# ka9q/ka9q-radio

Hardware: NVIDIA H100
Metric: input Msamples/s through forward+filter+inverse at N channels (higher is better)
Workload: dtype f32

## Files before the change

include/ka9q_gpu.h:

```cpp
#ifndef KA9Q_GPU_H
#define KA9Q_GPU_H 1
#include <stddef.h>
#include <stdint.h>

#ifdef __cplusplus
extern "C" {
#endif

enum kgpu_type { KGPU_COMPLEX = 1, KGPU_REAL = 2 };
enum kgpu_format {
  KGPU_FMT_F32 = 0,
  KGPU_FMT_I16 = 1
};
enum kgpu_chan_flags {
  KGPU_CHAN_ISB = 1,
  KGPU_CHAN_BEAM = 4
};

typedef struct kgpu_master kgpu_master;
typedef struct kgpu_bank kgpu_bank;

struct kgpu_ingest_stats {
  unsigned long long energy;
  unsigned int clips;
// ... 136 lines not shown
int kgpu_bank_run_one_ex(kgpu_bank *b, int idx, const void *d_spec, void *d_out, float *d_power , void *stream);
int kgpu_bank_noise(kgpu_bank *b, const void *d_spec, int nblocks, double samprate, double *d_n0, void *stream);

int kgpu_bank_fm_front(kgpu_bank *b, const void *d_out, long out_pitch, int nblocks, float *d_baseband, double *d_stats, void *stream);

int kgpu_bank_commit(kgpu_bank *b, void *stream);
int kgpu_use_static_kernels(int on);
int kgpu_use_cols_tma(int on);
int kgpu_cols_tma_fits(int L, int M, int in_type, int fmt, const void *d_in);
int kgpu_use_fused_forward(int on);
int kgpu_fused_forward_fits(int L, int M, int in_type, int fmt, const void *d_in);
int kgpu_fused_forward_options(int lead, int discard);
int kgpu_fused_shape(int *out);
int kgpu_fused_schedule(int nblocks, int lead, int ticket, int *out);
long kgpu_fused_discards(int blk, int idx, long *lines, long max);

int kgpu_plan_radices(int len, int *radices, int max);
int kgpu_plan_split(long n, int *n1, int *n2);
int kgpu_plan_radices_ex(int len, int *radices, int max);
int kgpu_plan_split_ex(long n, int *n1, int *n2);

int kgpu_multicast_copy(const void *d_src, void *mc_dst, unsigned long long bytes, int nctas, void *stream);

typedef struct kgpu_spectrum kgpu_spectrum;
kgpu_spectrum *kgpu_spectrum_create(int fft_n, int in_type, int bin_count);
int kgpu_spectrum_set_window(kgpu_spectrum *s, float const *window);
int kgpu_spectrum_run(kgpu_spectrum *s, const void *d_ring, long ring_samples, long end, int fmt, float scale,
                      const struct kgpu_scale_change *d_chg, int nchg, long long end_index, int derandomize, int shift, int fft_avg, double overlap, float *d_bins, void *stream);
int kgpu_spectrum_run_narrow(kgpu_spectrum *s, const void *d_ring, long ring_size, long ring_idx, int fft_avg,
                             double overlap, float *d_bins, int *fft_avg_used, void *stream);
// ... 12 lines not shown
```

ka9q_radio_b200/capi.py:

```python
from __future__ import annotations

import ctypes as C
import os
import subprocess
from pathlib import Path

PKG = Path(__file__).resolve().parent
LIB_PATH = PKG / "libka9qgpu.so"

KGPU_COMPLEX, KGPU_REAL = 1, 2
KGPU_FMT_F32, KGPU_FMT_I16 = 0, 1
KGPU_RAW_U8, KGPU_RAW_S8 = 1, 2
KGPU_RAW_S16, KGPU_RAW_U16, KGPU_RAW_SC16Q11 = 3, 4, 5
KGPU_RAW_F32, KGPU_RAW_CF32, KGPU_RAW_CF32_CNRMF, KGPU_RAW_CF32_FSCALE = 6, 7, 8, 9
KGPU_CHAN_ISB = 1
KGPU_CHAN_BEAM = 4

_lib = None


class KgpuError(RuntimeError):
    pass


# ... 81 lines not shown
    L.kgpu_bank_block_counter.restype = l
    L.kgpu_bank_run_ex.argtypes = [vp, vp, i, vp, l, vp, vp]
    L.kgpu_bank_run_one_ex.argtypes = [vp, i, vp, vp, vp, vp]
    L.kgpu_bank_noise.argtypes = [vp, vp, i, d, vp, vp]
    L.kgpu_bank_fm_front.argtypes = [vp, vp, l, i, vp, vp, vp]
    L.kgpu_use_static_kernels.argtypes = [i]
    L.kgpu_use_cols_tma.argtypes = [i]
    L.kgpu_cols_tma_fits.argtypes = [i, i, i, i, vp]
    L.kgpu_use_fused_forward.argtypes = [i]
    L.kgpu_fused_forward_fits.argtypes = [i, i, i, i, vp]
    L.kgpu_fused_forward_options.argtypes = [i, i]
    L.kgpu_fused_shape.argtypes = [vp]
    L.kgpu_fused_schedule.argtypes = [i, i, i, vp]
    L.kgpu_fused_discards.argtypes = [i, i, vp, l]
    L.kgpu_fused_discards.restype = l
    L.kgpu_profile_enable.argtypes = [i]
    L.kgpu_profile_name.argtypes = [i]
    L.kgpu_profile_name.restype = C.c_char_p
    L.kgpu_profile_get.argtypes = [i, vp, vp]
    L.kgpu_plan_radices.argtypes = [i, vp, i]
    L.kgpu_plan_split.argtypes = [l, vp, vp]
    L.kgpu_plan_radices_ex.argtypes = [i, vp, i]
    L.kgpu_plan_split_ex.argtypes = [l, vp, vp]
    L.kgpu_multicast_copy.argtypes = [vp, vp, C.c_ulonglong, i, vp]
    L.kgpu_algorithmic_bytes.argtypes = [vp, vp, i]
    L.kgpu_algorithmic_bytes.restype = d
    L.kgpu_spectrum_create.restype = vp
    L.kgpu_spectrum_create.argtypes = [i, i, i]
    L.kgpu_spectrum_set_window.argtypes = [vp, vp]
    L.kgpu_spectrum_run.argtypes = [vp, vp, l, l, i, f, vp, i, C.c_longlong, i, i, i, d, vp, vp]
# ... 369 lines not shown
```

ka9q_radio_b200/csrc/fft_static.cuh:

```cuda
#pragma once
#include "fft_radix.cuh"

namespace kfft {

template <int LEN, int... RS> struct SPlan {
  static constexpr int len = LEN;
  static constexpr int nst = sizeof...(RS);
  static constexpr int rad_arr[sizeof...(RS) > 0 ? sizeof...(RS) : 1] = {RS...};
  static constexpr int rad(int i) { return rad_arr[i]; }
  static constexpr int nsub(int i) {
    int n = LEN;
    for (int k = 0; k < i; k++) n /= rad_arr[k];
    return n;
  }
  static constexpr int stride(int i) { return nsub(i) / rad_arr[i]; }
  static constexpr int tw_off(int i) {
    int o = 0;
    for (int k = 0; k < i; k++)
      if (stride(k) > 1) o += (rad_arr[k] - 1) * stride(k);
    return o;
  }
  static constexpr bool valid() {
    int p = 1;
    for (int k = 0; k < nst; k++) p *= rad_arr[k];
// ... 104 lines not shown
}
__device__ __forceinline__ void mbar_fence_init() { asm volatile("fence.mbarrier_init.release.cluster;" ::: "memory"); }
__device__ __forceinline__ void mbar_expect_tx(uint64_t *bar, uint32_t bytes) {
  asm volatile("mbarrier.arrive.expect_tx.shared::cta.b64 _, [%0], %1;" ::"r"(smem_u32(bar)), "r"(bytes) : "memory");
}
__device__ __forceinline__ void bulk_g2s(void *dst, void const *src, uint32_t bytes, uint64_t *bar) {
  asm volatile("cp.async.bulk.shared::cluster.global.mbarrier::complete_tx::bytes [%0], [%1], %2, [%3];" ::"r"(smem_u32(dst)),
               "l"(src), "r"(bytes), "r"(smem_u32(bar))
               : "memory");
}
__device__ __forceinline__ void tensor_g2s_3d(void *dst, void const *map, int x, int y, int z, uint64_t *bar) {
  asm volatile("cp.async.bulk.tensor.3d.shared::cluster.global.tile.mbarrier::complete_tx::bytes [%0], [%1, {%2, %3, %4}], [%5];"
               ::"r"(smem_u32(dst)), "l"(map), "r"(x), "r"(y), "r"(z), "r"(smem_u32(bar))
               : "memory");
}
__device__ __forceinline__ void fence_proxy_async_global() { asm volatile("fence.proxy.async.global;" ::: "memory"); }
__device__ __forceinline__ void discard_l2_line(void *p) { asm volatile("discard.global.L2 [%0], 128;" ::"l"(p) : "memory"); }
__device__ __forceinline__ void mbar_wait(uint64_t *bar, uint32_t parity) {
  asm volatile(
      "{\n\t.reg .pred p;\n\t"
      "WAIT_%=:\n\t"
      "mbarrier.try_wait.parity.shared::cta.b64 p, [%0], %1;\n\t"
      "@p bra DONE_%=;\n\t"
      "bra WAIT_%=;\n\t"
      "DONE_%=:\n\t}" ::"r"(smem_u32(bar)),
      "r"(parity)
      : "memory");
}

}
// ... 1 lines not shown
```

ka9q_radio_b200/csrc/fwd_fused.cuh:

```cuda
#pragma once
#include "fwd_cols_r36.cuh"
#include "static_kernels_v2.cuh"

namespace kfft {

struct FusedShape {
  static constexpr int N1 = 1296, N2 = 1250;
  static constexpr int TILES = (N2 + 7) / 8;
  static constexpr int NC = (TILES + 1) / 2;
  static constexpr int NR = (N1 / 2 + 1 + RowsV2Shape<true>::IPC - 1) / RowsV2Shape<true>::IPC;
  static constexpr int T = 2 * ColsR36Shape::T;
  static constexpr int RT = RowsV2Shape<true>::T;
  static constexpr size_t smem = 2 * ColsR36Shape::smem > RowsV2Shape<true>::smem ? 2 * ColsR36Shape::smem : RowsV2Shape<true>::smem;
  static constexpr int DEFAULT_LEAD = 40;
  static_assert(ColsR36Shape::smem % 16 == 0, "the second tile's memory 16-byte aligned");
  static_assert(T % 32 == 0 && ColsR36Shape::T % 32 == 0 && RT % 32 == 0, "whole warps per tile and per R item");
};

enum FusedKind : int { kFusedCol = 0, kFusedRow = 1 };
struct FusedItem {
  int kind, blk, idx;
};

__host__ __device__ __forceinline__ FusedItem fused_item(int t, int nblocks, int lead) {
  using F = FusedShape;
  if (t < F::NC) return {kFusedCol, 0, t};
  t -= F::NC;
  int const b = t / (F::NR + F::NC), p = t - b * (F::NR + F::NC);
// ... 10 lines not shown
  int discard;
};

__device__ __forceinline__ void red_release_gpu_add(unsigned *p, unsigned v) {
  asm volatile("red.release.gpu.global.add.u32 [%0], %1;" ::"l"(p), "r"(v) : "memory");
}
__device__ __forceinline__ unsigned ld_acquire_gpu(unsigned const *p) {
  unsigned v;
  asm volatile("ld.acquire.gpu.global.u32 %0, [%1];" : "=r"(v) : "l"(p) : "memory");
  return v;
}

template <int FMT>
__global__ void __launch_bounds__(FusedShape::T, 1)
    fwd_fused_r36_v2(Pass1Args const a1, ColsR36Tables const t1, Pass2Args const a2, FwdTables const t2, FusedArgs const f,
                     const __grid_constant__ CUtensorMap tmap) {
  using F = FusedShape;
  extern __shared__ __align__(16) unsigned char smem_raw[];
  __shared__ __align__(8) uint64_t bars[RowsV2Shape<true>::COLS];
  __shared__ __align__(8) uint64_t tbar[2];
  __shared__ int s_ticket;
  int const tid = threadIdx.x;
  if (tid == 0) s_ticket = (int)atomicAdd(f.ctr, 1u);
  __syncthreads();
  FusedItem const it = fused_item(s_ticket, f.nblocks, f.lead);
  if (it.kind == kFusedCol) {
    int const h = tid >= ColsR36Shape::T, tile = 2 * it.idx + h;
    if (tile < F::TILES)
      fwd_cols_r36_body<FMT, F::N2, true>(a1, t1, &tmap, smem_raw + h * ColsR36Shape::smem, tbar[h], tid - h * ColsR36Shape::T,
                                           tile * 8, it.blk, [h] {
                                             asm volatile("bar.sync %0, %1;" ::"r"(1 + h), "n"(ColsR36Shape::T) : "memory");
// ... 6 lines not shown
    return;
  }
  if (tid >= F::RT) return;
  auto sync = [] { asm volatile("bar.sync 3, %0;" ::"n"(F::RT) : "memory"); };
  auto sync_or = [](int p) {
    int r;
    asm volatile("{\n\t.reg .pred q, o;\n\tsetp.ne.s32 q, %1, 0;\n\tbar.red.or.pred o, 3, %2, q;\n\tselp.s32 %0, 1, 0, o;\n\t}"
                 : "=r"(r)
                 : "r"(p), "n"(F::RT)
                 : "memory");
    return r;
  };
  if (tid == 0)
    while (ld_acquire_gpu(f.ctr + 1 + it.blk) < (unsigned)F::NC) __nanosleep(64);
  sync();
  fwd_rows_v2_body<true, F::N1, true, true>(a2, t2, smem_raw, bars, tbar[0], tid, it.blk, it.idx * RowsV2Shape<true>::IPC,
                                            sync, sync_or, f.discard);
}

}
```

ka9q_radio_b200/csrc/fwd_kernels.cuh:

```cuda
#pragma once
#include "fft_tile.cuh"

namespace kfft {

constexpr int kTile = 8;
constexpr int kFwdThreads = kTile * 32;

struct IngestStats {
  unsigned long long energy;
  unsigned int clips;
  unsigned int pad;
};

struct Pass1Args {
  void const *in;
  long hop;
  int n1, n2;
  long nc;
  int plan;
  int pitch;
  float scale;
  int derandomize;
  long first_new;
  float2 *mid;
// ... 146 lines not shown
  else it.kind = kRowEmpty, it.row_a = it.row_b = 0;
  return it;
}

struct Pass2Args {
  float2 const *mid;
  int n1, n2;
  long nc;
  int plan;
  int pitch;
  int real_split;
  float2 const *rootD;
  float2 *spec;
  long spec_stride;
  int mid_ld;
};

__global__ void __launch_bounds__(kFwdThreads, 2) fwd_rows_kernel(Pass2Args const a) {
  TilePlan const &pl = c_plans[a.plan];
#define KFFT_ROWS_EXT false
#include "fwd_rows_body.cuh"
#undef KFFT_ROWS_EXT
}
__global__ void __launch_bounds__(kFwdThreads, 2) fwd_rows_ext(Pass2Args const a, __grid_constant__ TilePlan const pl) {
#define KFFT_ROWS_EXT true
#include "fwd_rows_body.cuh"
#undef KFFT_ROWS_EXT
}

struct NotchDev {
// ... 34 lines not shown
```

ka9q_radio_b200/csrc/kgpu.cu:

```cuda
#include <cuda_runtime.h>
#include <cudaTypedefs.h>
#include <math.h>
#include <stdarg.h>
#include <stdio.h>
#include <stdlib.h>
#include <string.h>
#include <algorithm>
#include <complex>
#include <atomic>
#include <map>
#include <mutex>
#include <string>
#include <vector>

#include "../../include/ka9q_gpu.h"
#include "chan_kernels.cuh"
#include "chan_huge.cuh"
#include "chan_wide.cuh"
#include "fwd_kernels.cuh"
#include "noise_kernel.cuh"
#include "plan.cuh"
#include "static_kernels.cuh"
#include "static_kernels_v2.cuh"
#include "fwd_cols_r36.cuh"
// ... 30 lines not shown
  }
  return v != 0;
}
static std::atomic<int> g_fused{-1};
static std::atomic<int> g_fused_lead{FusedShape::DEFAULT_LEAD}, g_fused_discard{0};
extern "C" int kgpu_use_fused_forward(int on) {
  g_fused.store(on != 0);
  return 0;
}
static bool fused_on() {
  int v = g_fused.load();
  if (v < 0) {
    char const *e = getenv("KA9Q_FUSED_FWD");
    g_fused.compare_exchange_strong(v, (e && *e) ? (atoi(e) != 0) : 1);
    v = g_fused.load();
  }
  return v != 0;
}

static int fail(char const *fmt, ...) {
  char buf[512];
  va_list ap;
  va_start(ap, fmt);
  vsnprintf(buf, sizeof buf, fmt, ap);
  va_end(ap);
  g_err = buf;
  return -1;
}
#define CUDA_OK(expr)                                                                    \
  do {                                                                                   \
// ... 893 lines not shown
  size_t smem1 = 0, smem2 = 0;
  bool ext = false;
  TilePlan xplan1{}, xplan2{};
  kgpu_master *bs = nullptr;
  Bluestein blue;
  StreamBuf b_in, b_out;
  int b_chunk = 0;
  NotchDev *d_notch = nullptr;
  int n_notch = 0;
  int notch_sequential = 0;
};

using ColsR36Fn = void (*)(Pass1Args, ColsR36Tables);
using ColsR36TmaFn = void (*)(Pass1Args, ColsR36Tables, CUtensorMap);
using Cols2sFn = void (*)(Pass1Args, Cols2sTables);
using RowsV2Fn = void (*)(Pass2Args, FwdTables);
using Cols2s = Cols2sShape<25, 32>;
using Rows2s = Rows2sShape<25, 25>;
static ColsR36Fn cols_r36_kernel(kgpu_master const *m, int f) {
  static ColsR36Fn const k[2][3] = {{fwd_cols_r36<0, 0>, fwd_cols_r36<1, 0>, fwd_cols_r36<2, 0>},
                                    {fwd_cols_r36<0, 1250>, fwd_cols_r36<1, 1250>, fwd_cols_r36<2, 1250>}};
  return k[m->n2c == 1250][f];
}
static ColsR36TmaFn cols_r36_tma_kernel(kgpu_master const *m, int f) {
  static ColsR36TmaFn const k[2][3] = {{fwd_cols_r36_tma<0, 0>, fwd_cols_r36_tma<1, 0>, fwd_cols_r36_tma<2, 0>},
                                       {fwd_cols_r36_tma<0, 1250>, fwd_cols_r36_tma<1, 1250>, fwd_cols_r36_tma<2, 1250>}};
  return k[m->n2c == 1250][f];
}
static Cols2sFn cols_2s_kernel(int f) {
  static Cols2sFn const k[3] = {fwd_cols_2s<0, 25, 32>, fwd_cols_2s<1, 25, 32>, fwd_cols_2s<2, 25, 32>};
  return k[f];
}
static RowsV2Fn rows_v2_kernel(kgpu_master const *m) {
  if (m->in_type == KGPU_REAL) return m->halved ? fwd_rows_v2<true, 1296, true> : fwd_rows_v2<true, 0, false>;
  return m->n1c ? fwd_rows_v2<false, 1296, false> : fwd_rows_v2<false, 0, false>;
}
static bool fused_pair(kgpu_master const *m) {
  return m->in_type == KGPU_REAL && m->cols == COLS_R36 && m->rows == ROWS_V2 && m->halved && m->n2c == FusedShape::N2 &&
         m->n1c == FusedShape::N1 && m->mid_ld % 16 == 0;
}
using FusedFn = void (*)(Pass1Args, ColsR36Tables, Pass2Args, FwdTables, FusedArgs, CUtensorMap);
static FusedFn fused_kernel(int f) {
  static FusedFn const k[3] = {fwd_fused_r36_v2<0>, fwd_fused_r36_v2<1>, fwd_fused_r36_v2<2>};
  return k[f];
}
static int rows_v2_threads(kgpu_master const *m) { return m->in_type == KGPU_REAL ? RowsV2Shape<true>::T : RowsV2Shape<false>::T; }
static size_t rows_v2_smem(kgpu_master const *m) {
  return m->in_type == KGPU_REAL ? RowsV2Shape<true>::smem : RowsV2Shape<false>::smem;
}

static int upload(float2 **d, std::vector<float2> const &v) {
  CUDA_OK(cudaMalloc(d, sizeof(float2) * v.size()));
  CUDA_OK(cudaMemcpy(*d, v.data(), sizeof(float2) * v.size(), cudaMemcpyHostToDevice));
  return 0;
}

static int bluestein_upload(Bluestein *b) {
  if (upload(&b->d_b, bluestein_bspec(b->n, b->P)) == 0) return 0;
  cudaFree(b->d_b);
  b->d_b = nullptr;
  return -1;
}

// ... 78 lines not shown
    std::vector<float2> t0((size_t)Cols2s::TW0, make_float2(0.f, 0.f)), tA((size_t)n2 * RA),
        tB((size_t)(n2 + 8) * Cols2s::NP1, make_float2(0.f, 0.f)), r0((size_t)Rows2s::TW0, make_float2(0.f, 0.f));
    for (int e = 0; e < Cols2s::NP0; e++)
      for (int j = 0; j < RB; j++) t0[(size_t)e * RB + j] = root((long)j * Pow<RA>::exponent(e), n1);
    for (long c = 0; c < n2; c++) {
      for (int t = 0; t < RA; t++) tA[(size_t)c * RA + t] = root(c * t, m->nc);
      for (int e = 0; e < Cols2s::NP1; e++) tB[(size_t)c * Cols2s::NP1 + e] = root(c * RA * Pow<RB>::exponent(e), m->nc);
    }
    for (int e = 0; e < Rows2s::NP0; e++)
      for (int j = 0; j < RD; j++) r0[(size_t)e * RD + j] = root((long)j * Pow<RC>::exponent(e), n2);
    if (upload(&m->d_tw0, t0) || upload(&m->d_twA, tA) || upload(&m->d_twB, tB) || upload(&m->d_rtw0, r0)) return -1;
    for (int f = 0; f < 3; f++)
      if (allow_smem((const void *)cols_2s_kernel(f), Cols2s::smem)) return -1;
    if (allow_smem((const void *)fwd_rows_2s<25, 25>, Rows2s::smem)) return -1;
  }
  if (m->rows == ROWS_V2 && allow_smem((const void *)rows_v2_kernel(m), rows_v2_smem(m))) return -1;
  if (fused_pair(m))
    for (int f = 0; f < 3; f++)
      if (allow_smem((const void *)fused_kernel(f), FusedShape::smem)) return -1;
  if (m->ext) {
    if (allow_smem((const void *)fwd_cols_ext<0>, m->smem1) || allow_smem((const void *)fwd_cols_ext<1>, m->smem1) ||
        allow_smem((const void *)fwd_rows_ext, m->smem2))
      return -1;
  } else if (allow_smem((const void *)fwd_cols_kernel<0>, m->smem1) || allow_smem((const void *)fwd_cols_kernel<1>, m->smem1) ||
             allow_smem((const void *)fwd_rows_kernel, m->smem2)) {
    return -1;
  }
  return 0;
}

extern "C" void kgpu_master_destroy(kgpu_master *m) {
  if (!m) return;
  if (m->ext) {
    free_tile_plan(m->xplan1);
// ... 231 lines not shown
extern "C" long kgpu_fused_discards(int blk, int idx, long *lines, long max) {
  using S = RowsV2Shape<true>;
  if (blk < 0 || idx < 0 || idx >= FusedShape::NR || max < 0) return fail("kgpu_fused_discards: bad arguments");
  int const ld = (FusedShape::N2 + 15) / 16 * 16;
  long n = 0;
  for (int col = 0; col < S::COLS; col++) {
    RowItem const it = row_item(idx * S::IPC + (col >> 1), FusedShape::N1, true);
    int const row = (col & 1) == 0 ? (it.kind != kRowEmpty ? it.row_a : -1) : (it.kind == kRowPair ? it.row_b : -1);
    if (row < 0) continue;
    for (int l = 0; l < mid_row_lines(ld); l++, n++)
      if (lines && n < max) lines[n] = mid_line(blk, FusedShape::N1, row, ld, l);
  }
  return n;
}

static int cols_tma_map(kgpu_master const *m, void const *d_in, int fmt, int nblocks, CUtensorMap *map) {
  static PFN_cuTensorMapEncodeTiled const encode = [] {
    void *fn = nullptr;
    cudaDriverEntryPointQueryResult q;
    if (cudaGetDriverEntryPoint("cuTensorMapEncodeTiled", &fn, cudaEnableDefault, &q) != cudaSuccess ||
        q != cudaDriverEntryPointSuccess)
      fn = nullptr;
    return (PFN_cuTensorMapEncodeTiled)fn;
  }();
  if (!encode) return fail("kgpu_forward: the driver has no cuTensorMapEncodeTiled");
  bool const i16 = fmt == KGPU_FMT_I16;
  cuuint64_t const n1 = (cuuint64_t)m->sp.n1, n2 = (cuuint64_t)m->sp.n2;
  cuuint64_t const hop = (cuuint64_t)(m->in_type == KGPU_REAL ? m->L / 2 : m->L);
  cuuint64_t const dim[3] = {2 * n2, i16 ? n1 / 2 : n1, (cuuint64_t)nblocks};
  cuuint64_t const stride[2] = {8 * n2, hop * (i16 ? 4 : 8)};
  cuuint32_t const box[3] = {(cuuint32_t)(i16 ? ColsR36Tma::I16_BOX_WORDS : 16), ColsR36Tma::BOX_ROWS, 1};
  cuuint32_t const unit[3] = {1, 1, 1};
  CUresult const r = encode(map, i16 ? CU_TENSOR_MAP_DATA_TYPE_UINT32 : CU_TENSOR_MAP_DATA_TYPE_FLOAT32, 3, const_cast<void *>(d_in),
                            dim, stride, box, unit, CU_TENSOR_MAP_INTERLEAVE_NONE, CU_TENSOR_MAP_SWIZZLE_NONE,
                            CU_TENSOR_MAP_L2_PROMOTION_L2_128B, CU_TENSOR_MAP_FLOAT_OOB_FILL_NONE);
  if (r != CUDA_SUCCESS) return fail("kgpu_forward: cuTensorMapEncodeTiled failed (%d)", (int)r);
  return 0;
}

static Pass2Args rows_args(kgpu_master const *m, Pass1Args const &a1, void *d_spec) {
  Pass2Args a2;
  a2.mid = a1.mid;
  a2.n1 = m->sp.n1;
  a2.n2 = m->sp.n2;
  a2.nc = m->nc;
  a2.plan = m->plan2;
  a2.pitch = m->pitch2;
  a2.real_split = (m->in_type == KGPU_REAL);
  a2.rootD = m->d_rootD;
  a2.spec = (float2 *)d_spec;
  a2.spec_stride = m->spec_stride;
  a2.mid_ld = a1.mid_ld;
  return a2;
}

static int fused_span(kgpu_master *m, const void *d_in, int fmt, int f, int nblocks, void *d_spec, cudaStream_t st,
                      Pass1Args const &a1) {
  using F = FusedShape;
  size_t const ctr_bytes = sizeof(unsigned) * (size_t)(1 + nblocks);
  if (grow(m->fused_ctr, ctr_bytes, st, "kgpu_forward")) return -1;
  CUtensorMap map;
  if (cols_tma_map(m, d_in, fmt, nblocks, &map)) return -1;
  FusedArgs fa;
  fa.ctr = (unsigned *)m->fused_ctr.p;
  fa.nblocks = nblocks;
  fa.lead = g_fused_lead.load();
  fa.discard = g_fused_discard.load();
  CUDA_OK(cudaMemsetAsync(fa.ctr, 0, ctr_bytes, st));
  {
    ProfScope ps(K_FWD_FUSED, st);
    fused_kernel(f)<<<(unsigned)(nblocks * (F::NC + F::NR)), F::T, F::smem, st>>>(a1, ColsR36Tables{m->d_tw0, m->d_twA, m->d_twB},
                                                                       rows_args(m, a1, d_spec), FwdTables{m->d_rootC}, fa, map);
  }
  g_launches++;
  CUDA_OK(cudaGetLastError());
  return 0;
}

static int forward_span(kgpu_master *m, const void *d_in, int fmt, float scale, int derandomize, int nblocks, void *d_spec,
                        void *d_stats, cudaStream_t st, float2 *mid) {
  bool const use_static = g_static_on.load() != 0;
  ColsKernel const cols = use_static ? m->cols : COLS_GENERIC;
  RowsKernel const rows = use_static ? m->rows : ROWS_GENERIC;
  Pass1Args a1;
  a1.in = d_in;
  a1.hop = (m->in_type == KGPU_REAL) ? m->L / 2 : m->L;
  a1.n1 = m->sp.n1;
// ... 23 lines not shown
          if (cols_tma_map(m, d_in, fmt, nblocks, &map)) return -1;
          cols_r36_tma_kernel(m, f)<<<g1, ColsR36Shape::T, ColsR36Shape::smem, st>>>(a1, ColsR36Tables{m->d_tw0, m->d_twA, m->d_twB}, map);
        } else {
          cols_r36_kernel(m, f)<<<g1, ColsR36Shape::T, ColsR36Shape::smem, st>>>(a1, ColsR36Tables{m->d_tw0, m->d_twA, m->d_twB});
        }
        break;
      case COLS_GENERIC:
        if (m->ext && f) fwd_cols_ext<1><<<g1, kFwdThreads, m->smem1, st>>>(a1, m->xplan1);
        else if (m->ext) fwd_cols_ext<0><<<g1, kFwdThreads, m->smem1, st>>>(a1, m->xplan1);
        else if (f) fwd_cols_kernel<1><<<g1, kFwdThreads, m->smem1, st>>>(a1);
        else fwd_cols_kernel<0><<<g1, kFwdThreads, m->smem1, st>>>(a1);
        break;
    }
  }
  g_launches++;
  Pass2Args const a2 = rows_args(m, a1, d_spec);
  dim3 const g2((unsigned)(rows == ROWS_GENERIC ? m->n_item_ctas : m->n_rows_ctas), (unsigned)nblocks);
  {
    ProfScope ps(K_FWD_ROWS, st);
    switch (rows) {
      case ROWS_2S:
        fwd_rows_2s<25, 25><<<g2, Rows2s::T, Rows2s::smem, st>>>(a2, m->d_rtw0);
        break;
      case ROWS_V2:
        rows_v2_kernel(m)<<<g2, rows_v2_threads(m), rows_v2_smem(m), st>>>(a2, FwdTables{m->d_rootC});
        break;
      case ROWS_GENERIC:
        if (m->ext) fwd_rows_ext<<<g2, kFwdThreads, m->smem2, st>>>(a2, m->xplan2);
        else fwd_rows_kernel<<<g2, kFwdThreads, m->smem2, st>>>(a2);
        break;
    }
  }
  g_launches++;
  CUDA_OK(cudaGetLastError());
  return 0;
}

static int bluestein_conv(kgpu_master *im, Bluestein const &b, float2 *a, int rows, float2 *y, cudaStream_t st) {
  if (kgpu_forward(im, a, KGPU_FMT_F32, 1.0f, 0, rows, y, nullptr, st) != 0) return -1;
  {
// ... 1336 lines not shown
```

ka9q_radio_b200/csrc/static_kernels_v2.cuh:

```cuda
#pragma once
#include "static_kernels.cuh"

namespace kfft {

__device__ __forceinline__ void unpack_i16(int raw, int &lo, int &hi) {
  asm("prmt.b32 %0, %1, 0, 0x9910;" : "=r"(lo) : "r"(raw));
  hi = raw >> 16;
}
__device__ __forceinline__ float i32_to_f32(int v) {
  float f;
  asm("cvt.rn.f32.s32 %0, %1;" : "=f"(f) : "r"(v));
  return f;
}

template <bool REAL_SPLIT>
struct RowsV2Shape {
  using P = SPlan<1250, 10, 25, 5>;
  static constexpr int N2 = 1250, PITCH = 1250, GT = 256, SKEW = 2;
  static constexpr int NG = REAL_SPLIT ? 2 : 1, T = GT * NG, COLS = 8 * NG;
  static constexpr int IPC = REAL_SPLIT ? COLS / 2 : COLS;
  static constexpr int TW = (static_tw_count<P>() + 1) & ~1;
  static constexpr int TILE = COLS * PITCH + (NG - 1) * SKEW;
  static constexpr size_t smem = sizeof(float2) * (size_t)(TILE + TW);
  static __host__ __device__ constexpr int col_off(int c) { return c * PITCH + (c >> 3) * SKEW; }
};

__device__ constexpr float kRowsTw0[3][4][2] = {
    {{9.870916009e-01f, -1.601568460e-01f}, {9.486995935e-01f, -3.161789477e-01f}, {8.000617623e-01f, -5.999176502e-01f}, {2.801976204e-01f, -9.599423409e-01f}},
    {{9.486995935e-01f, -3.161789477e-01f}, {8.000617623e-01f, -5.999176502e-01f}, {2.801976204e-01f, -9.599423409e-01f}, {-8.429785967e-01f, -5.379471183e-01f}},
    {{8.858151436e-01f, -4.640382826e-01f}, {5.693368912e-01f, -8.221042752e-01f}, {-3.517109454e-01f, -9.361086488e-01f}, {-7.525988221e-01f, 6.584793329e-01f}},
};

__host__ __device__ constexpr int mid_row_lines(int mid_ld) { return mid_ld * 8 / 128; }
__host__ __device__ constexpr long mid_line(int blk, int n1, int row, int mid_ld, int l) {
  return ((long)blk * n1 + row) * mid_row_lines(mid_ld) + l;
}

template <bool REAL_SPLIT, int N1C, bool HALVED, bool FUSED, class Sync, class SyncOr>
__device__ __forceinline__ void fwd_rows_v2_body(Pass2Args const &a, FwdTables const &tb, unsigned char *smem_raw,
                                                 uint64_t *bars, uint64_t &tbar, int tid, int blk, int item0,
                                                 Sync const &sync, SyncOr const &sync_or, bool discard = false) {
  using S = RowsV2Shape<REAL_SPLIT>;
  using P = typename S::P;
  constexpr int N2 = S::N2, T = S::T, GT = S::GT, COLS = S::COLS, IPC = S::IPC;
  constexpr int R0 = 10, S0 = 125, R1 = 25, NSUB1 = 125, S1 = 5, R2 = 5;
  float2 *tile = reinterpret_cast<float2 *>(smem_raw);
  float2 *s_tw = tile + S::TILE;
  TilePlan const &pl = c_plans[a.plan];
  int const lane = tid & 31, warp = tid >> 5;
  int const n1 = N1C ? N1C : a.n1;
  auto row_of = [&](int col) -> int {
    RowItem const it = row_item(item0 + (REAL_SPLIT ? col >> 1 : col), n1, REAL_SPLIT);
    if (REAL_SPLIT) {
      if ((col & 1) == 0) return it.kind != kRowEmpty ? it.row_a : -1;
      return it.kind == kRowPair ? it.row_b : -1;
    }
// ... 63 lines not shown
    float2 const *tw1 = s_tw + P::tw_off(1);
#pragma unroll 1
    for (int u = ul; u < N2 / R1; u += GT / 8) {
      int const b = u / S1, j = u - b * S1;
      float2 *p = mycol + b * NSUB1 + j;
      float2 x[R1];
#pragma unroll
      for (int m = 0; m < R1; m++) x[m] = p[m * S1];
      Dft<R1, false>::run(x);
#pragma unroll
      for (int t = 1; t < R1; t++) x[t] = cmul(x[t], tw1[(t - 1) * S1 + j]);
#pragma unroll
      for (int t = 0; t < R1; t++) p[t * S1] = x[t];
    }
  }
  constexpr int UQ = T / IPC;
  int const i = tid % IPC, uq = tid / IPC;
  RowItem const it = row_item(item0 + i, n1, REAL_SPLIT);
  float2 rootC = make_float2(1.f, 0.f), rd[4];
  bool self_item = false;
  if (REAL_SPLIT) {
    self_item = it.kind == kRowSelf0 || it.kind == kRowSelfMid;
    if (it.kind == kRowPair) rootC = __ldg(tb.rootC + it.row_a);
#pragma unroll
    for (int q = 0; q < 4; q++) {
      int const u = uq + UQ * q;
      int const t0 = u / 25, t1 = u - t0 * 25;
      rd[q] = (it.kind == kRowPair && u < N2 / R2) ? __ldg(a.rootD + t0 + 10 * t1) : make_float2(1.f, 0.f);
    }
  }
  int const has_self = sync_or(self_item);

  float2 *spec = a.spec + (long)blk * a.spec_stride;
  float const hf = HALVED ? 1.0f : 0.5f;
  if (!REAL_SPLIT) {
    if (col_ok) {
      float2 *dst = spec + row_of(c);
#pragma unroll 1
      for (int u = ul; u < N2 / R2; u += GT / 8) {
        int const t0 = u / 25, t1 = u - t0 * 25;
        int const kb = t0 + 10 * t1;
        float2 const *p = mycol + u * R2;
        float2 x[R2];
#pragma unroll
        for (int m = 0; m < R2; m++) x[m] = p[m];
        Dft<R2, false>::run(x);
        float2 *d = dst + (long)n1 * kb;
#pragma unroll
        for (int t = 0; t < R2; t++) d[(long)n1 * 250 * t] = x[t];
      }
    }
    return;
  }
  int const nc = N1C ? N1C * N2 : (int)a.nc;
  if (it.kind == kRowPair) {
    float2 const *ca = tile + S::col_off(2 * i), *cb = tile + S::col_off(2 * i + 1);
#pragma unroll
    for (int q = 0; q < 4; q++) {
      int const u = uq + UQ * q;
      if (u >= N2 / R2) break;
      int const t0 = u / 25, t1 = u - t0 * 25;
      int const kb = t0 + 10 * t1;
      float2 const wkb = cmul(rootC, rd[q]);
      float2 za[R2], zb[R2];
      float2 const *pa = ca + u * R2, *pb = cb + (N2 / R2 - 1 - u) * R2;
      float2 *pk = spec + (it.row_a + n1 * kb), *pm = spec + (nc - it.row_a - n1 * kb);
#pragma unroll
      for (int m = 0; m < R2; m++) {
        za[m] = pa[m];
        zb[m] = pb[m];
      }
      Dft<R2, false>::run(za);
      Dft<R2, false>::run(zb);
#pragma unroll
      for (int t = 0; t < R2; t++) {
        float2 const A = za[t], B = zb[R2 - 1 - t];
        float2 const w = (t == 0) ? wkb : cmul(wkb, wroot<10>(t));
        float2 const E = HALVED ? make_float2(A.x + B.x, A.y - B.y) : make_float2(0.5f * (A.x + B.x), 0.5f * (A.y - B.y));
        float2 const O = HALVED ? make_float2(A.x - B.x, A.y + B.y) : make_float2(0.5f * (A.x - B.x), 0.5f * (A.y + B.y));
        float2 const Pp = cmul(w, O);
        pk[(long)n1 * 250 * t] = make_float2(E.x + Pp.y, E.y - Pp.x);
        pm[-(long)n1 * 250 * t] = make_float2(E.x - Pp.y, -(E.y + Pp.x));
      }
    }
  }
  if (!has_self) return;
  for (int s = 0; s < IPC; s++) {
    RowItem const its = row_item(item0 + s, n1, true);
    if (its.kind != kRowSelf0 && its.kind != kRowSelfMid) continue;
    float2 *col = tile + S::col_off(2 * s);
    for (int u = tid; u < N2 / R2; u += T) {
      float2 x[R2];
#pragma unroll
      for (int m = 0; m < R2; m++) x[m] = col[u * R2 + m];
      Dft<R2, false>::run(x);
#pragma unroll
      for (int m = 0; m < R2; m++) col[u * R2 + m] = x[m];
// ... 10 lines not shown
    for (int k2 = tid; k2 < kend; k2 += T) {
      int const k2m = self0 ? (k2 == 0 ? 0 : N2 - k2) : N2 - 1 - k2;
      float2 const A = col[static_slot<P>(k2)], B = col[static_slot<P>(k2m)];
      float2 const w = cmul(rC, __ldg(a.rootD + k2));
      float2 const E = make_float2(hf * (A.x + B.x), hf * (A.y - B.y));
      float2 const O = make_float2(hf * (A.x - B.x), hf * (A.y + B.y));
      float2 const Pp = cmul(w, O);
      int const k = its.row_a + n1 * k2;
      spec[k] = make_float2(E.x + Pp.y, E.y - Pp.x);
      if (nc - k != k) spec[nc - k] = make_float2(E.x - Pp.y, -(E.y + Pp.x));
    }
  }
}

template <bool REAL_SPLIT, int N1C = 0, bool HALVED = false>
__global__ void __launch_bounds__(RowsV2Shape<REAL_SPLIT>::T, REAL_SPLIT ? 1 : 2) fwd_rows_v2(Pass2Args const a, FwdTables const tb) {
  extern __shared__ __align__(16) unsigned char smem_raw[];
  __shared__ __align__(8) uint64_t bars[RowsV2Shape<REAL_SPLIT>::COLS];
  __shared__ __align__(8) uint64_t tbar;
  fwd_rows_v2_body<REAL_SPLIT, N1C, HALVED, false>(a, tb, smem_raw, bars, tbar, threadIdx.x, gridDim.y - 1 - blockIdx.y,
                                                   blockIdx.x * RowsV2Shape<REAL_SPLIT>::IPC, [] { __syncthreads(); },
                                                   [](int p) { return __syncthreads_or(p); });
}

template <class P, bool OSC = false>
__global__ void __launch_bounds__(kChanWarps * 32) chan_v2(ChanArgs const a) {
  static_assert(P::nst == 2, "two-stage plans only");
  __shared__ __align__(8) uint64_t bars[kChanWarps];
  __shared__ __align__(8) uint64_t tbar;
  using S = StaticChan<P>;
  constexpr int NS = S::NS, R0 = P::rad(0), R1 = P::rad(1), S0 = NS / R0;
  static_assert(S0 == R1, "plan shape");
  S s;
  if (!static_prologue<P>(a, bars, tbar, s)) return;
  ChanDesc const &d = s.d;
// ... 52 lines not shown
```

Baseline: 104,100.

## Store forward rows-pass low-half spectrum via TMA bulk tensor stores

```diff
diff --git a/include/ka9q_gpu.h b/include/ka9q_gpu.h
--- a/include/ka9q_gpu.h
+++ b/include/ka9q_gpu.h
@@ -174,6 +174,8 @@
 int kgpu_fused_shape(int *out);
 int kgpu_fused_schedule(int nblocks, int lead, int ticket, int *out);
 long kgpu_fused_discards(int blk, int idx, long *lines, long max);
+int kgpu_use_rows_tma_store(int on);
+int kgpu_rows_store_box(int item, int round, int *out);
 
 int kgpu_plan_radices(int len, int *radices, int max);
 int kgpu_plan_split(long n, int *n1, int *n2);
diff --git a/ka9q_radio_b200/capi.py b/ka9q_radio_b200/capi.py
--- a/ka9q_radio_b200/capi.py
+++ b/ka9q_radio_b200/capi.py
@@ -119,6 +119,8 @@
     L.kgpu_fused_schedule.argtypes = [i, i, i, vp]
     L.kgpu_fused_discards.argtypes = [i, i, vp, l]
     L.kgpu_fused_discards.restype = l
+    L.kgpu_use_rows_tma_store.argtypes = [i]
+    L.kgpu_rows_store_box.argtypes = [i, i, vp]
     L.kgpu_profile_enable.argtypes = [i]
     L.kgpu_profile_name.argtypes = [i]
     L.kgpu_profile_name.restype = C.c_char_p
diff --git a/ka9q_radio_b200/csrc/fft_static.cuh b/ka9q_radio_b200/csrc/fft_static.cuh
--- a/ka9q_radio_b200/csrc/fft_static.cuh
+++ b/ka9q_radio_b200/csrc/fft_static.cuh
@@ -142,6 +142,15 @@
                ::"r"(smem_u32(dst)), "l"(map), "r"(x), "r"(y), "r"(z), "r"(smem_u32(bar))
                : "memory");
 }
+__device__ __forceinline__ void tensor_s2g_4d(void const *map, void const *src, int x, int y, int z, int w) {
+  asm volatile("cp.async.bulk.tensor.4d.global.shared::cta.bulk_group [%0, {%1, %2, %3, %4}], [%5];" ::"l"(map), "r"(x), "r"(y),
+               "r"(z), "r"(w), "r"(smem_u32(src))
+               : "memory");
+}
+__device__ __forceinline__ void bulk_commit() { asm volatile("cp.async.bulk.commit_group;" ::: "memory"); }
+__device__ __forceinline__ void bulk_wait_read_all() { asm volatile("cp.async.bulk.wait_group.read 0;" ::: "memory"); }
+__device__ __forceinline__ void bulk_wait_all() { asm volatile("cp.async.bulk.wait_group 0;" ::: "memory"); }
+__device__ __forceinline__ void fence_proxy_async_shared() { asm volatile("fence.proxy.async.shared::cta;" ::: "memory"); }
 __device__ __forceinline__ void fence_proxy_async_global() { asm volatile("fence.proxy.async.global;" ::: "memory"); }
 __device__ __forceinline__ void discard_l2_line(void *p) { asm volatile("discard.global.L2 [%0], 128;" ::"l"(p) : "memory"); }
 __device__ __forceinline__ void mbar_wait(uint64_t *bar, uint32_t parity) {
diff --git a/ka9q_radio_b200/csrc/fwd_fused.cuh b/ka9q_radio_b200/csrc/fwd_fused.cuh
--- a/ka9q_radio_b200/csrc/fwd_fused.cuh
+++ b/ka9q_radio_b200/csrc/fwd_fused.cuh
@@ -12,6 +12,7 @@
   static constexpr int T = 2 * ColsR36Shape::T;
   static constexpr int RT = RowsV2Shape<true>::T;
   static constexpr size_t smem = 2 * ColsR36Shape::smem > RowsV2Shape<true>::smem ? 2 * ColsR36Shape::smem : RowsV2Shape<true>::smem;
+  static constexpr size_t smem_store = smem > RowsV2Shape<true>::smem_store ? smem : RowsV2Shape<true>::smem_store;
   static constexpr int DEFAULT_LEAD = 40;
   static_assert(ColsR36Shape::smem % 16 == 0, "the second tile's memory 16-byte aligned");
   static_assert(T % 32 == 0 && ColsR36Shape::T % 32 == 0 && RT % 32 == 0, "whole warps per tile and per R item");
@@ -52,7 +53,7 @@
 template <int FMT>
 __global__ void __launch_bounds__(FusedShape::T, 1)
     fwd_fused_r36_v2(Pass1Args const a1, ColsR36Tables const t1, Pass2Args const a2, FwdTables const t2, FusedArgs const f,
-                     const __grid_constant__ CUtensorMap tmap) {
+                     const __grid_constant__ CUtensorMap tmap, const __grid_constant__ CUtensorMap smap) {
   using F = FusedShape;
   extern __shared__ __align__(16) unsigned char smem_raw[];
   __shared__ __align__(8) uint64_t bars[RowsV2Shape<true>::COLS];
@@ -89,7 +90,7 @@
   if (tid == 0)
     while (ld_acquire_gpu(f.ctr + 1 + it.blk) < (unsigned)F::NC) __nanosleep(64);
   sync();
-  fwd_rows_v2_body<true, F::N1, true, true>(a2, t2, smem_raw, bars, tbar[0], tid, it.blk, it.idx * RowsV2Shape<true>::IPC,
+  fwd_rows_v2_body<true, F::N1, true, true>(a2, t2, &smap, smem_raw, bars, tbar[0], tid, it.blk, it.idx * RowsV2Shape<true>::IPC,
                                             sync, sync_or, f.discard);
 }
 
diff --git a/ka9q_radio_b200/csrc/fwd_kernels.cuh b/ka9q_radio_b200/csrc/fwd_kernels.cuh
--- a/ka9q_radio_b200/csrc/fwd_kernels.cuh
+++ b/ka9q_radio_b200/csrc/fwd_kernels.cuh
@@ -184,6 +184,7 @@
   float2 *spec;
   long spec_stride;
   int mid_ld;
+  int spec_tma = 0;
 };
 
 __global__ void __launch_bounds__(kFwdThreads, 2) fwd_rows_kernel(Pass2Args const a) {
diff --git a/ka9q_radio_b200/csrc/kgpu.cu b/ka9q_radio_b200/csrc/kgpu.cu
--- a/ka9q_radio_b200/csrc/kgpu.cu
+++ b/ka9q_radio_b200/csrc/kgpu.cu
@@ -68,6 +68,20 @@
     char const *e = getenv("KA9Q_FUSED_FWD");
     g_fused.compare_exchange_strong(v, (e && *e) ? (atoi(e) != 0) : 1);
     v = g_fused.load();
+  }
+  return v != 0;
+}
+static std::atomic<int> g_rows_tma_store{-1};
+extern "C" int kgpu_use_rows_tma_store(int on) {
+  g_rows_tma_store.store(on != 0);
+  return 0;
+}
+static bool rows_tma_store_on() {
+  int v = g_rows_tma_store.load();
+  if (v < 0) {
+    char const *e = getenv("KA9Q_ROWS_TMA_STORE");
+    g_rows_tma_store.compare_exchange_strong(v, (e && *e) ? (atoi(e) != 0) : 1);
+    v = g_rows_tma_store.load();
   }
   return v != 0;
 }
@@ -991,7 +1005,7 @@
 using ColsR36Fn = void (*)(Pass1Args, ColsR36Tables);
 using ColsR36TmaFn = void (*)(Pass1Args, ColsR36Tables, CUtensorMap);
 using Cols2sFn = void (*)(Pass1Args, Cols2sTables);
-using RowsV2Fn = void (*)(Pass2Args, FwdTables);
+using RowsV2Fn = void (*)(Pass2Args, FwdTables, CUtensorMap);
 using Cols2s = Cols2sShape<25, 32>;
 using Rows2s = Rows2sShape<25, 25>;
 static ColsR36Fn cols_r36_kernel(kgpu_master const *m, int f) {
@@ -1016,7 +1030,7 @@
   return m->in_type == KGPU_REAL && m->cols == COLS_R36 && m->rows == ROWS_V2 && m->halved && m->n2c == FusedShape::N2 &&
          m->n1c == FusedShape::N1 && m->mid_ld % 16 == 0;
 }
-using FusedFn = void (*)(Pass1Args, ColsR36Tables, Pass2Args, FwdTables, FusedArgs, CUtensorMap);
+using FusedFn = void (*)(Pass1Args, ColsR36Tables, Pass2Args, FwdTables, FusedArgs, CUtensorMap, CUtensorMap);
 static FusedFn fused_kernel(int f) {
   static FusedFn const k[3] = {fwd_fused_r36_v2<0>, fwd_fused_r36_v2<1>, fwd_fused_r36_v2<2>};
   return k[f];
@@ -1024,6 +1038,10 @@
 static int rows_v2_threads(kgpu_master const *m) { return m->in_type == KGPU_REAL ? RowsV2Shape<true>::T : RowsV2Shape<false>::T; }
 static size_t rows_v2_smem(kgpu_master const *m) {
   return m->in_type == KGPU_REAL ? RowsV2Shape<true>::smem : RowsV2Shape<false>::smem;
+}
+static bool rows_store_pair(kgpu_master const *m) { return m->in_type == KGPU_REAL && m->rows == ROWS_V2 && m->halved && m->n1c == 1296; }
+static bool rows_store_fits(kgpu_master const *m, void const *d_spec) {
+  return rows_store_pair(m) && (uintptr_t)d_spec % 16 == 0 && 8 * m->spec_stride % 16 == 0;
 }
 
 static int upload(float2 **d, std::vector<float2> const &v) {
@@ -1132,10 +1150,12 @@
       if (allow_smem((const void *)cols_2s_kernel(f), Cols2s::smem)) return -1;
     if (allow_smem((const void *)fwd_rows_2s<25, 25>, Rows2s::smem)) return -1;
   }
-  if (m->rows == ROWS_V2 && allow_smem((const void *)rows_v2_kernel(m), rows_v2_smem(m))) return -1;
+  if (m->rows == ROWS_V2 &&
+      allow_smem((const void *)rows_v2_kernel(m), rows_store_pair(m) ? RowsV2Shape<true>::smem_store : rows_v2_smem(m)))
+    return -1;
   if (fused_pair(m))
     for (int f = 0; f < 3; f++)
-      if (allow_smem((const void *)fused_kernel(f), FusedShape::smem)) return -1;
+      if (allow_smem((const void *)fused_kernel(f), FusedShape::smem_store)) return -1;
   if (m->ext) {
     if (allow_smem((const void *)fwd_cols_ext<0>, m->smem1) || allow_smem((const void *)fwd_cols_ext<1>, m->smem1) ||
         allow_smem((const void *)fwd_rows_ext, m->smem2))
@@ -1397,7 +1417,16 @@
   return n;
 }
 
-static int cols_tma_map(kgpu_master const *m, void const *d_in, int fmt, int nblocks, CUtensorMap *map) {
+extern "C" int kgpu_rows_store_box(int item, int round, int *out) {
+  using S = RowsV2Shape<true>;
+  if (item < 0 || item >= FusedShape::NR || round < 0 || round >= S::ROUNDS || !out) return fail("kgpu_rows_store_box: bad arguments");
+  RowsStoreBox const b = rows_store_box(item, round);
+  int const v[5] = {S::IPC, S::UQ, S::R2, b.k1, b.kb};
+  for (int k = 0; k < 5; k++) out[k] = v[k];
+  return rows_store_item(FusedShape::N1, item) ? 1 : 0;
+}
+
+static PFN_cuTensorMapEncodeTiled tensor_map_encoder() {
   static PFN_cuTensorMapEncodeTiled const encode = [] {
     void *fn = nullptr;
     cudaDriverEntryPointQueryResult q;
@@ -1406,6 +1435,10 @@
       fn = nullptr;
     return (PFN_cuTensorMapEncodeTiled)fn;
   }();
+  return encode;
+}
+static int cols_tma_map(kgpu_master const *m, void const *d_in, int fmt, int nblocks, CUtensorMap *map) {
+  PFN_cuTensorMapEncodeTiled const encode = tensor_map_encoder();
   if (!encode) return fail("kgpu_forward: the driver has no cuTensorMapEncodeTiled");
   bool const i16 = fmt == KGPU_FMT_I16;
   cuuint64_t const n1 = (cuuint64_t)m->sp.n1, n2 = (cuuint64_t)m->sp.n2;
@@ -1418,6 +1451,21 @@
                             dim, stride, box, unit, CU_TENSOR_MAP_INTERLEAVE_NONE, CU_TENSOR_MAP_SWIZZLE_NONE,
                             CU_TENSOR_MAP_L2_PROMOTION_L2_128B, CU_TENSOR_MAP_FLOAT_OOB_FILL_NONE);
   if (r != CUDA_SUCCESS) return fail("kgpu_forward: cuTensorMapEncodeTiled failed (%d)", (int)r);
+  return 0;
+}
+
+static int rows_store_map(kgpu_master const *m, void *d_spec, int nblocks, CUtensorMap *map) {
+  using S = RowsV2Shape<true>;
+  PFN_cuTensorMapEncodeTiled const encode = tensor_map_encoder();
+  if (!encode) return fail("kgpu_forward: the driver has no cuTensorMapEncodeTiled");
+  cuuint64_t const n1 = (cuuint64_t)m->sp.n1, nkb = S::N2 / S::R2;
+  cuuint64_t const dim[4] = {2 * n1, nkb, (cuuint64_t)S::R2, (cuuint64_t)nblocks};
+  cuuint64_t const stride[3] = {8 * n1, 8 * n1 * nkb, 8 * (cuuint64_t)m->spec_stride};
+  cuuint32_t const box[4] = {2 * (cuuint32_t)S::IPC, (cuuint32_t)S::UQ, (cuuint32_t)S::R2, 1};
+  cuuint32_t const unit[4] = {1, 1, 1, 1};
+  CUresult const r = encode(map, CU_TENSOR_MAP_DATA_TYPE_FLOAT32, 4, d_spec, dim, stride, box, unit, CU_TENSOR_MAP_INTERLEAVE_NONE,
+                            CU_TENSOR_MAP_SWIZZLE_NONE, CU_TENSOR_MAP_L2_PROMOTION_NONE, CU_TENSOR_MAP_FLOAT_OOB_FILL_NONE);
+  if (r != CUDA_SUCCESS) return fail("kgpu_forward: cuTensorMapEncodeTiled failed for the spectrum (%d)", (int)r);
   return 0;
 }
 
@@ -1442,8 +1490,11 @@
   using F = FusedShape;
   size_t const ctr_bytes = sizeof(unsigned) * (size_t)(1 + nblocks);
   if (grow(m->fused_ctr, ctr_bytes, st, "kgpu_forward")) return -1;
-  CUtensorMap map;
+  CUtensorMap map, smap{};
   if (cols_tma_map(m, d_in, fmt, nblocks, &map)) return -1;
+  Pass2Args a2 = rows_args(m, a1, d_spec);
+  a2.spec_tma = rows_tma_store_on() && rows_store_fits(m, d_spec);
+  if (a2.spec_tma && rows_store_map(m, d_spec, nblocks, &smap)) return -1;
   FusedArgs fa;
   fa.ctr = (unsigned *)m->fused_ctr.p;
   fa.nblocks = nblocks;
@@ -1452,8 +1503,8 @@
   CUDA_OK(cudaMemsetAsync(fa.ctr, 0, ctr_bytes, st));
   {
     ProfScope ps(K_FWD_FUSED, st);
-    fused_kernel(f)<<<(unsigned)(nblocks * (F::NC + F::NR)), F::T, F::smem, st>>>(a1, ColsR36Tables{m->d_tw0, m->d_twA, m->d_twB},
-                                                                       rows_args(m, a1, d_spec), FwdTables{m->d_rootC}, fa, map);
+    fused_kernel(f)<<<(unsigned)(nblocks * (F::NC + F::NR)), F::T, a2.spec_tma ? F::smem_store : F::smem, st>>>(
+        a1, ColsR36Tables{m->d_tw0, m->d_twA, m->d_twB}, a2, FwdTables{m->d_rootC}, fa, map, smap);
   }
   g_launches++;
   CUDA_OK(cudaGetLastError());
@@ -1507,7 +1558,10 @@
     }
   }
   g_launches++;
-  Pass2Args const a2 = rows_args(m, a1, d_spec);
+  Pass2Args a2 = rows_args(m, a1, d_spec);
+  CUtensorMap smap{};
+  a2.spec_tma = rows == ROWS_V2 && rows_tma_store_on() && rows_store_fits(m, d_spec);
+  if (a2.spec_tma && rows_store_map(m, d_spec, nblocks, &smap)) return -1;
   dim3 const g2((unsigned)(rows == ROWS_GENERIC ? m->n_item_ctas : m->n_rows_ctas), (unsigned)nblocks);
   {
     ProfScope ps(K_FWD_ROWS, st);
@@ -1516,7 +1570,8 @@
         fwd_rows_2s<25, 25><<<g2, Rows2s::T, Rows2s::smem, st>>>(a2, m->d_rtw0);
         break;
       case ROWS_V2:
-        rows_v2_kernel(m)<<<g2, rows_v2_threads(m), rows_v2_smem(m), st>>>(a2, FwdTables{m->d_rootC});
+        rows_v2_kernel(m)<<<g2, rows_v2_threads(m), a2.spec_tma ? RowsV2Shape<true>::smem_store : rows_v2_smem(m), st>>>(
+            a2, FwdTables{m->d_rootC}, smap);
         break;
       case ROWS_GENERIC:
         if (m->ext) fwd_rows_ext<<<g2, kFwdThreads, m->smem2, st>>>(a2, m->xplan2);
diff --git a/ka9q_radio_b200/csrc/static_kernels_v2.cuh b/ka9q_radio_b200/csrc/static_kernels_v2.cuh
--- a/ka9q_radio_b200/csrc/static_kernels_v2.cuh
+++ b/ka9q_radio_b200/csrc/static_kernels_v2.cuh
@@ -23,7 +23,22 @@
   static constexpr int TILE = COLS * PITCH + (NG - 1) * SKEW;
   static constexpr size_t smem = sizeof(float2) * (size_t)(TILE + TW);
   static __host__ __device__ constexpr int col_off(int c) { return c * PITCH + (c >> 3) * SKEW; }
+  static constexpr int UQ = T / IPC, R2 = 5, ROUNDS = (N2 / R2 + UQ - 1) / UQ;
+  static constexpr int BOX = R2 * UQ * IPC;
+  static constexpr size_t smem_store = smem + 128 + sizeof(float2) * (size_t)BOX;
 };
+
+__host__ __device__ __forceinline__ bool rows_store_item(int n1, int item) {
+  constexpr int IPC = RowsV2Shape<true>::IPC;
+  return row_item(item * IPC, n1, true).kind == kRowPair && row_item(item * IPC + IPC - 1, n1, true).kind == kRowPair;
+}
+struct RowsStoreBox {
+  int k1, kb;
+};
+__host__ __device__ __forceinline__ RowsStoreBox rows_store_box(int item, int q) {
+  using S = RowsV2Shape<true>;
+  return {S::IPC * item, S::UQ * q};
+}
 
 __device__ constexpr float kRowsTw0[3][4][2] = {
     {{9.870916009e-01f, -1.601568460e-01f}, {9.486995935e-01f, -3.161789477e-01f}, {8.000617623e-01f, -5.999176502e-01f}, {2.801976204e-01f, -9.599423409e-01f}},
@@ -37,9 +52,9 @@
 }
 
 template <bool REAL_SPLIT, int N1C, bool HALVED, bool FUSED, class Sync, class SyncOr>
-__device__ __forceinline__ void fwd_rows_v2_body(Pass2Args const &a, FwdTables const &tb, unsigned char *smem_raw,
-                                                 uint64_t *bars, uint64_t &tbar, int tid, int blk, int item0,
-                                                 Sync const &sync, SyncOr const &sync_or, bool discard = false) {
+__device__ __forceinline__ void fwd_rows_v2_body(Pass2Args const &a, FwdTables const &tb, CUtensorMap const *smap,
+                                                 unsigned char *smem_raw, uint64_t *bars, uint64_t &tbar, int tid, int blk,
+                                                 int item0, Sync const &sync, SyncOr const &sync_or, bool discard = false) {
   using S = RowsV2Shape<REAL_SPLIT>;
   using P = typename S::P;
   constexpr int N2 = S::N2, T = S::T, GT = S::GT, COLS = S::COLS, IPC = S::IPC;
@@ -133,7 +148,7 @@
       for (int t = 0; t < R1; t++) p[t * S1] = x[t];
     }
   }
-  constexpr int UQ = T / IPC;
+  constexpr int UQ = S::UQ;
   int const i = tid % IPC, uq = tid / IPC;
   RowItem const it = row_item(item0 + i, n1, REAL_SPLIT);
   float2 rootC = make_float2(1.f, 0.f), rd[4];
@@ -143,9 +158,8 @@
     if (it.kind == kRowPair) rootC = __ldg(tb.rootC + it.row_a);
 #pragma unroll
     for (int q = 0; q < 4; q++) {
-      int const u = uq + UQ * q;
-      int const t0 = u / 25, t1 = u - t0 * 25;
-      rd[q] = (it.kind == kRowPair && u < N2 / R2) ? __ldg(a.rootD + t0 + 10 * t1) : make_float2(1.f, 0.f);
+      int const kb = uq + UQ * q;
+      rd[q] = (it.kind == kRowPair && kb < N2 / R2) ? __ldg(a.rootD + kb) : make_float2(1.f, 0.f);
     }
   }
   int const has_self = sync_or(self_item);
@@ -172,34 +186,77 @@
     return;
   }
   int const nc = N1C ? N1C * N2 : (int)a.nc;
+  float2 const *ca = tile + S::col_off(2 * i), *cb = tile + S::col_off(2 * i + 1);
+  auto split = [&](int kb, float2 rdq, float2 (&lo)[R2], float2 (&hi)[R2]) {
+    int const t0 = kb % 10, u = 25 * t0 + kb / 10;
+    float2 const wkb = cmul(rootC, rdq);
+    float2 za[R2], zb[R2];
+    float2 const *pa = ca + u * R2, *pb = cb + (N2 / R2 - 1 - u) * R2;
+#pragma unroll
+    for (int m = 0; m < R2; m++) {
+      za[m] = pa[m];
+      zb[m] = pb[m];
+    }
+    Dft<R2, false>::run(za);
+    Dft<R2, false>::run(zb);
+#pragma unroll
+    for (int t = 0; t < R2; t++) {
+      float2 const A = za[t], B = zb[R2 - 1 - t];
+      float2 const w = (t == 0) ? wkb : cmul(wkb, wroot<10>(t));
+      float2 const E = HALVED ? make_float2(A.x + B.x, A.y - B.y) : make_float2(0.5f * (A.x + B.x), 0.5f * (A.y - B.y));
+      float2 const O = HALVED ? make_float2(A.x - B.x, A.y + B.y) : make_float2(0.5f * (A.x - B.x), 0.5f * (A.y + B.y));
+      float2 const Pp = cmul(w, O);
+      lo[t] = make_float2(E.x + Pp.y, E.y - Pp.x);
+      hi[t] = make_float2(E.x - Pp.y, -(E.y + Pp.x));
+    }
+  };
+  if constexpr (REAL_SPLIT && N1C % 8 == 0 && N1C != 0) {
+    if (a.spec_tma && rows_store_item(n1, item0 / IPC)) {
+      unsigned char *const st_raw = smem_raw + S::smem;
+      float2 *const sd = reinterpret_cast<float2 *>(st_raw + ((0u - smem_u32(st_raw)) & 127u));
+#pragma unroll
+      for (int q = 0; q < S::ROUNDS; q++) {
+        int const kb = uq + UQ * q;
+        bool const live = kb < N2 / R2;
+        float2 lo[R2], hi[R2];
+        if (live) {
+          split(kb, rd[q], lo, hi);
+          float2 *pm = spec + (nc - it.row_a - n1 * kb);
+#pragma unroll
+          for (int t = 0; t < R2; t++) pm[-(long)n1 * 250 * t] = hi[t];
+        }
+        if (q > 0) {
+          if (tid == 0) bulk_wait_read_all();
+          sync();
+        }
+        if (live) {
+#pragma unroll
+          for (int t = 0; t < R2; t++) sd[(t * UQ + uq) * IPC + i] = lo[t];
+        }
+        fence_proxy_async_shared();
+        sync();
+        if (tid == 0) {
+          RowsStoreBox const bx = rows_store_box(item0 / IPC, q);
+          tensor_s2g_4d(smap, sd, 2 * bx.k1, bx.kb, 0, blk);
+          bulk_commit();
+        }
+      }
+      if (tid == 0) bulk_wait_all();
+      return;
+    }
+  }
   if (it.kind == kRowPair) {
-    float2 const *ca = tile + S::col_off(2 * i), *cb = tile + S::col_off(2 * i + 1);
 #pragma unroll
     for (int q = 0; q < 4; q++) {
-      int const u = uq + UQ * q;
-      if (u >= N2 / R2) break;
-      int const t0 = u / 25, t1 = u - t0 * 25;
-      int const kb = t0 + 10 * t1;
-      float2 const wkb = cmul(rootC, rd[q]);
-      float2 za[R2], zb[R2];
-      float2 const *pa = ca + u * R2, *pb = cb + (N2 / R2 - 1 - u) * R2;
+      int const kb = uq + UQ * q;
+      if (kb >= N2 / R2) break;
+      float2 lo[R2], hi[R2];
+      split(kb, rd[q], lo, hi);
       float2 *pk = spec + (it.row_a + n1 * kb), *pm = spec + (nc - it.row_a - n1 * kb);
 #pragma unroll
-      for (int m = 0; m < R2; m++) {
-        za[m] = pa[m];
-        zb[m] = pb[m];
-      }
-      Dft<R2, false>::run(za);
-      Dft<R2, false>::run(zb);
-#pragma unroll
       for (int t = 0; t < R2; t++) {
-        float2 const A = za[t], B = zb[R2 - 1 - t];
-        float2 const w = (t == 0) ? wkb : cmul(wkb, wroot<10>(t));
-        float2 const E = HALVED ? make_float2(A.x + B.x, A.y - B.y) : make_float2(0.5f * (A.x + B.x), 0.5f * (A.y - B.y));
-        float2 const O = HALVED ? make_float2(A.x - B.x, A.y + B.y) : make_float2(0.5f * (A.x - B.x), 0.5f * (A.y + B.y));
-        float2 const Pp = cmul(w, O);
-        pk[(long)n1 * 250 * t] = make_float2(E.x + Pp.y, E.y - Pp.x);
-        pm[-(long)n1 * 250 * t] = make_float2(E.x - Pp.y, -(E.y + Pp.x));
+        pk[(long)n1 * 250 * t] = lo[t];
+        pm[-(long)n1 * 250 * t] = hi[t];
       }
     }
   }
@@ -240,11 +297,12 @@
 }
 
 template <bool REAL_SPLIT, int N1C = 0, bool HALVED = false>
-__global__ void __launch_bounds__(RowsV2Shape<REAL_SPLIT>::T, REAL_SPLIT ? 1 : 2) fwd_rows_v2(Pass2Args const a, FwdTables const tb) {
+__global__ void __launch_bounds__(RowsV2Shape<REAL_SPLIT>::T, REAL_SPLIT ? 1 : 2)
+    fwd_rows_v2(Pass2Args const a, FwdTables const tb, const __grid_constant__ CUtensorMap smap) {
   extern __shared__ __align__(16) unsigned char smem_raw[];
   __shared__ __align__(8) uint64_t bars[RowsV2Shape<REAL_SPLIT>::COLS];
   __shared__ __align__(8) uint64_t tbar;
-  fwd_rows_v2_body<REAL_SPLIT, N1C, HALVED, false>(a, tb, smem_raw, bars, tbar, threadIdx.x, gridDim.y - 1 - blockIdx.y,
+  fwd_rows_v2_body<REAL_SPLIT, N1C, HALVED, false>(a, tb, &smap, smem_raw, bars, tbar, threadIdx.x, gridDim.y - 1 - blockIdx.y,
                                                    blockIdx.x * RowsV2Shape<REAL_SPLIT>::IPC, [] { __syncthreads(); },
                                                    [](int p) { return __syncthreads_or(p); });
 }
```

After: 104,000 (median of 6 runs). No clear change (-0.1%).
